# mathwrx/Decouple-and-Couple_Learning_in_Multi-Modal_Brain_Tumor_Segmentation

Hardware: AMD Instinct MI355X
Metric: training volumes/sec (4x128^3) (higher is better)
Workload: dtype bf16x3 forward (split-bf16 MFMA operands hi.hi+hi.lo+lo.hi: logits within 1e-3 of the fp32 reference) / bf16 data-gradient / bf16 weight-gradient MFMA operands; f32 accumulate, f32 storage, f32 master weights; 1 GPU; configs[1]: 1xMI355X, batch 2 per GPU, 4-modality 128^3 synthetic BraTS patches; fwd + softmax_dice + 4 sub-region/edge losses + bwd + Adam(amsgrad); random-init weights, dropout on; global_batch=2, parallelism=dp1, precision=bf16x3, dgrad_precision=bf16, wgrad_precision=bf16, mode=plan

## Files before the change

decouple-and-couple_learning_in_multi-modal_brain_tumor_segmentation_amd/csrc/attn.hip:

```cpp
#include "common.h"

#define AT_D 64
#define AT_TMAX 144
#define AT_QT 32
#define AT_LDK 68
#define AT_LDS 148

struct AttnArgs {
  const float* qkv; int64_t ld;
  float* o; int64_t ldo;
  const float* d_o;
  float* dqkv;
  int T, E, heads; float scale;
  const uint64_t* rng; uint64_t drop_off; float drop_p;
};

__device__ __forceinline__ f32x4 mfma4(float a, float b, f32x4 c) { return __builtin_amdgcn_mfma_f32_16x16x4f32(a, b, c, 0, 0, 0); }

__device__ __forceinline__ void at_load_tile(float* lds, const float* g, int64_t ld, int row0, int nrows, int valid_rows, int tid) {
  for (int i = tid; i < nrows * (AT_D / 4); i += 256) {
    const int r = i >> 4, c4 = (i & 15) * 4;
    float4 v = make_float4(0.f, 0.f, 0.f, 0.f);
    if (row0 + r < valid_rows) v = *reinterpret_cast<const float4*>(g + (int64_t)(row0 + r) * ld + c4);
    *reinterpret_cast<float4*>(lds + r * AT_LDK + c4) = v;
  }
}

__device__ __forceinline__ void at_scores(float* Ss, const float* As, const float* Bs, float alpha, int wave, int r, int kq) {
  for (int idx = wave; idx < 2 * 9; idx += 4) {
    const int mt = idx / 9, nt = idx % 9;
    f32x4 acc = {0.f, 0.f, 0.f, 0.f};
#pragma unroll
    for (int kk = 0; kk < AT_D / 4; ++kk)
      acc = mfma4(As[(mt * 16 + r) * AT_LDK + kk * 4 + kq], Bs[(nt * 16 + r) * AT_LDK + kk * 4 + kq], acc);
#pragma unroll
    for (int e = 0; e < 4; ++e) Ss[(mt * 16 + kq * 4 + e) * AT_LDS + nt * 16 + r] = acc[e] * alpha;
  }
}

__global__ __launch_bounds__(256) void attn_fwd_kernel(const AttnArgs a) {
  extern __shared__ float4 at_lds4[];
  float* Ks = reinterpret_cast<float*>(at_lds4);
  float* Vs = Ks + AT_TMAX * AT_LDK;
  float* Qs = Vs + AT_TMAX * AT_LDK;
// ... 30 lines not shown
        s[c] = p;
      }
    }
  }
  __syncthreads();
  for (int idx = wave; idx < 2 * 4; idx += 4) {
    const int mt = idx >> 2, nt = idx & 3;
    f32x4 acc = {0.f, 0.f, 0.f, 0.f};
#pragma unroll 4
    for (int kk = 0; kk < AT_TMAX / 4; ++kk)
      acc = mfma4(Ss[(mt * 16 + r) * AT_LDS + kk * 4 + kq], Vs[(kk * 4 + kq) * AT_LDK + nt * 16 + r], acc);
#pragma unroll
    for (int e = 0; e < 4; ++e) {
      const int q = q0 + mt * 16 + kq * 4 + e;
      if (q < T) a.o[((int64_t)z * T + q) * a.ldo + h * AT_D + nt * 16 + r] = acc[e];
    }
  }
}

__global__ __launch_bounds__(256) void attn_bwd_kernel(const AttnArgs a) {
  extern __shared__ float4 at_lds4[];
  float* Ks = reinterpret_cast<float*>(at_lds4);
  float* Vs = Ks + AT_TMAX * AT_LDK;
  float* Qs = Vs + AT_TMAX * AT_LDK;
  float* Gs = Qs + AT_QT * AT_LDK;
  float* Ss = Gs + AT_QT * AT_LDK;
  float* Ds = Ss + AT_QT * AT_LDS;
  const int tid = threadIdx.x, lane = tid & 63, wave = tid >> 6, r = lane & 15, kq = lane >> 4;
  const int zh = blockIdx.x, z = zh / a.heads, h = zh % a.heads, T = a.T;
  const float* base = a.qkv + (int64_t)z * T * a.ld + h * AT_D;
// ... 3 lines not shown
  at_load_tile(Vs, base + 2 * a.E, a.ld, 0, AT_TMAX, T, tid);
  f32x4 dk[9], dv[9];
#pragma unroll
  for (int i = 0; i < 9; ++i) { dk[i] = (f32x4){0.f, 0.f, 0.f, 0.f}; dv[i] = (f32x4){0.f, 0.f, 0.f, 0.f}; }
  const float inv_keep = a.drop_p > 0.f ? 1.f / (1.f - a.drop_p) : 1.f;
  for (int q0 = 0; q0 < T; q0 += AT_QT) {
    __syncthreads();
    at_load_tile(Qs, base, a.ld, q0, AT_QT, T, tid);
    at_load_tile(Gs, gbase, a.ldo, q0, AT_QT, T, tid);
    __syncthreads();
    at_scores(Ss, Qs, Ks, a.scale, wave, r, kq);
    at_scores(Ds, Gs, Vs, 1.f, wave, r, kq);
    __syncthreads();
    for (int rr = 0; rr < 8; ++rr) {
      const int row = wave * 8 + rr;
      float* s = Ss + row * AT_LDS; float* d = Ds + row * AT_LDS;
      const bool live = q0 + row < T;
      float v[3], g[3]; float mx = -INFINITY;
#pragma unroll
      for (int i = 0; i < 3; ++i) { const int c = lane + 64 * i; v[i] = c < T ? s[c] : -INFINITY; mx = fmaxf(mx, v[i]); }
      mx = wave_max(mx);
      float sum = 0.f;
#pragma unroll
      for (int i = 0; i < 3; ++i) { v[i] = (lane + 64 * i) < T ? expf(v[i] - mx) : 0.f; sum += v[i]; }
      const float inv = 1.f / wave_sum(sum);
      float dot = 0.f; float m[3];
#pragma unroll
      for (int i = 0; i < 3; ++i) {
        const int c = lane + 64 * i;
        v[i] *= inv; m[i] = 1.f;
        if (a.drop_p > 0.f && c < T)
          m[i] = cwf_rng_u01(a.rng, a.drop_off + ((uint64_t)zh * T + (q0 + row)) * T + c) >= a.drop_p ? inv_keep : 0.f;
        g[i] = c < T ? d[c] * m[i] : 0.f;
        dot += g[i] * v[i];
      }
      dot = wave_sum(dot);
#pragma unroll
      for (int i = 0; i < 3; ++i) {
        const int c = lane + 64 * i;
        if (c < AT_TMAX) {
          s[c] = live ? v[i] * m[i] : 0.f;
          d[c] = live ? v[i] * (g[i] - dot) * a.scale : 0.f;
        }
      }
    }
    __syncthreads();
#pragma unroll
    for (int mt = 0; mt < 9; ++mt) {
#pragma unroll
      for (int kk = 0; kk < AT_QT / 4; ++kk) {
        const int q = kk * 4 + kq;
        dv[mt] = mfma4(Ss[q * AT_LDS + mt * 16 + r], Gs[q * AT_LDK + wave * 16 + r], dv[mt]);
        dk[mt] = mfma4(Ds[q * AT_LDS + mt * 16 + r], Qs[q * AT_LDK + wave * 16 + r], dk[mt]);
      }
    }
    for (int idx = wave; idx < 2 * 4; idx += 4) {
      const int mt = idx >> 2, nt = idx & 3;
      f32x4 acc = {0.f, 0.f, 0.f, 0.f};
#pragma unroll 4
// ... 6 lines not shown
      }
    }
  }
#pragma unroll
  for (int mt = 0; mt < 9; ++mt)
#pragma unroll
    for (int e = 0; e < 4; ++e) {
      const int key = mt * 16 + kq * 4 + e;
      if (key < T) {
        dbase[(int64_t)key * a.ld + a.E + wave * 16 + r] = dk[mt][e];
        dbase[(int64_t)key * a.ld + 2 * a.E + wave * 16 + r] = dv[mt][e];
      }
    }
}

static int at_check(const float* qkv, int64_t ld, int Z, int T, int E, int heads) {
  if (!qkv || Z <= 0 || T <= 0 || heads <= 0 || E != heads * AT_D || ld < 3 * (int64_t)E || (ld & 3) || ((uintptr_t)qkv & 15)) return CWF_E_BADARG;
  if (T > AT_TMAX || (int64_t)Z * heads > 65535) return CWF_E_TOOLARGE;
  return 0;
}

static void at_set_lds(const void* fn, size_t bytes) {
  static bool done[2][64] = {};
  static const void* fns[2] = {nullptr, nullptr};
  int dev = 0; (void)hipGetDevice(&dev);
  int slot = (fns[0] == fn || fns[0] == nullptr) ? 0 : 1;
  fns[slot] = fn;
  if (dev < 0 || dev >= 64 || !done[slot][dev]) {
    (void)hipFuncSetAttribute(fn, hipFuncAttributeMaxDynamicSharedMemorySize, (int)bytes);
    if (dev >= 0 && dev < 64) done[slot][dev] = true;
  }
}

extern "C" int cwf_attn_fwd(const float* qkv, int64_t ld, float* o, int64_t ldo, int Z, int T, int E, int heads, float scale,
                            const uint64_t* rng, uint64_t drop_off, float drop_p, void* stream) {
  int rc = at_check(qkv, ld, Z, T, E, heads); if (rc) return rc;
  if (!o || ldo < E || (drop_p > 0.f && !rng) || drop_p < 0.f || drop_p >= 1.f) return CWF_E_BADARG;
  AttnArgs a{qkv, ld, o, ldo, nullptr, nullptr, T, E, heads, scale, rng, drop_off, drop_p};
  const size_t lds = sizeof(float) * (2 * AT_TMAX * AT_LDK + AT_QT * AT_LDK + AT_QT * AT_LDS);
  at_set_lds(reinterpret_cast<const void*>(&attn_fwd_kernel), lds);
  hipLaunchKernelGGL(attn_fwd_kernel, dim3(cdiv(T, AT_QT), Z * heads), dim3(256), lds, cwf_stream(stream), a);
  CWF_LAUNCH_CHECK();
  return 0;
}

extern "C" int cwf_attn_bwd(const float* qkv, int64_t ld, const float* d_o, int64_t ldo, float* dqkv, int Z, int T, int E, int heads,
                            float scale, const uint64_t* rng, uint64_t drop_off, float drop_p, void* stream) {
  int rc = at_check(qkv, ld, Z, T, E, heads); if (rc) return rc;
  if (!d_o || !dqkv || ldo < E || (ldo & 3) || ((uintptr_t)d_o & 15) || (drop_p > 0.f && !rng) || drop_p < 0.f || drop_p >= 1.f) return CWF_E_BADARG;
  AttnArgs a{qkv, ld, nullptr, ldo, d_o, dqkv, T, E, heads, scale, rng, drop_off, drop_p};
  const size_t lds = sizeof(float) * (2 * AT_TMAX * AT_LDK + 2 * AT_QT * AT_LDK + 2 * AT_QT * AT_LDS);
  at_set_lds(reinterpret_cast<const void*>(&attn_bwd_kernel), lds);
  hipLaunchKernelGGL(attn_bwd_kernel, dim3(Z * heads), dim3(256), lds, cwf_stream(stream), a);
  CWF_LAUNCH_CHECK();
  return 0;
}
```

decouple-and-couple_learning_in_multi-modal_brain_tumor_segmentation_amd/csrc/tokens.hip:

```cpp
#include "common.h"

__global__ void window_to_tokens_kernel(const float* __restrict__ x, int x_ldc, float* __restrict__ tok,
                                        int D, int H, int W, int C, int p0, int p1, int p2, int64_t total) {
  const int64_t idx = (int64_t)blockIdx.x * blockDim.x + threadIdx.x;
  if (idx >= total) return;
  const int E = C * p0 * p1 * p2;
  const int T = (D / p0) * (H / p1) * (W / p2);
  const int f = (int)(idx % E); const int64_t bt = idx / E;
  const int t = (int)(bt % T); const int b = (int)(bt / T);
  int ff = f; const int k = ff % p2; ff /= p2; const int j = ff % p1; ff /= p1; const int i = ff % p0; const int c = ff / p0;
  int tt = t; const int tw = tt % (W / p2); tt /= (W / p2); const int th = tt % (H / p1); const int td = tt / (H / p1);
  const int d = td * p0 + i, h = th * p1 + j, w = tw * p2 + k;
  tok[idx] = x[((((int64_t)b * D + d) * H + h) * W + w) * x_ldc + c];
}

__global__ void tokens_to_window_kernel(const float* __restrict__ tok, float* __restrict__ x, int x_ldc,
                                        int D, int H, int W, int C, int p0, int p1, int p2, int accumulate, int64_t total) {
  const int64_t idx = (int64_t)blockIdx.x * blockDim.x + threadIdx.x;
  if (idx >= total) return;
  const int c = (int)(idx % C); int64_t v = idx / C;
  const int w = (int)(v % W); v /= W; const int h = (int)(v % H); v /= H; const int d = (int)(v % D); const int b = (int)(v / D);
  const int E = C * p0 * p1 * p2;
  const int T = (D / p0) * (H / p1) * (W / p2);
  const int t = ((d / p0) * (H / p1) + h / p1) * (W / p2) + w / p2;
// ... 332 lines not shown
    float4 v = *reinterpret_cast<const float4*>(src + e);
    if (scat) *reinterpret_cast<float4*>(scat + o + e) = v;
    if (gated) {
      const float4 g = *reinterpret_cast<const float4*>(gate + b * gate_bs + e);
      v.x *= g.x; v.y *= g.y; v.z *= g.z; v.w *= g.w;
      *reinterpret_cast<float4*>(gated + o + e) = v;
    }
  }
}

struct ScatBwdArgs {
  const float* dgated; const float* dscat; const float* feats; const int32_t* inv; const int32_t* index;
  const float* rows; int64_t rows_ld, rows_bs; const float* gate; int64_t gate_bs; const float* dgate_extra; int64_t extra_bs;
  float* drows; int64_t drows_ld, drows_bs; float* dgate; int64_t dgate_bs; int T, k, E;
};
__global__ __launch_bounds__(1024) void scatter_bwd_kernel(const ScatBwdArgs a) {
  const int b = blockIdx.y, E = a.E, T = a.T;
  if ((int)blockIdx.x < a.k) {
    if (threadIdx.x >= 128) return;
    const int j = blockIdx.x;
    const int t = min(max(a.index[(int64_t)b * a.k + j], 0), T - 1);
    const int64_t o = ((int64_t)b * T + t) * E;
    for (int e = threadIdx.x * 4; e < E; e += 512) {
      float4 v = make_float4(0.f, 0.f, 0.f, 0.f);
      if (a.dgated) {
        const float4 d = *reinterpret_cast<const float4*>(a.dgated + o + e);
        const float4 g = *reinterpret_cast<const float4*>(a.gate + b * a.gate_bs + e);
        v = make_float4(d.x * g.x, d.y * g.y, d.z * g.z, d.w * g.w);
      }
      if (a.dscat) { const float4 s = *reinterpret_cast<const float4*>(a.dscat + o + e); v.x += s.x; v.y += s.y; v.z += s.z; v.w += s.w; }
      *reinterpret_cast<float4*>(a.drows + b * a.drows_bs + (int64_t)j * a.drows_ld + e) = v;
    }
    return;
  }
  __shared__ float red[16][64];
  const int w = threadIdx.x >> 6, lane = threadIdx.x & 63;
  const int c = (blockIdx.x - a.k) * 64 + lane;
  float acc = 0.f;
  if (c < E && a.dgated) {
    for (int t0 = w; t0 < T; t0 += 64) {
      float d[4], s[4];
#pragma unroll
      for (int u = 0; u < 4; ++u) {
        const int t = t0 + 16 * u;
        d[u] = 0.f; s[u] = 0.f;
        if (t < T) {
          const int j = a.inv[(int64_t)b * T + t];
          d[u] = a.dgated[((int64_t)b * T + t) * E + c];
          s[u] = j >= 0 ? a.rows[b * a.rows_bs + (int64_t)j * a.rows_ld + c] : a.feats[((int64_t)b * T + t) * E + c];
        }
      }
#pragma unroll
      for (int u = 0; u < 4; ++u) acc += d[u] * s[u];
    }
  }
  red[w][lane] = acc;
  __syncthreads();
  if (w == 0 && c < E) {
    float tsum = 0.f;
#pragma unroll
    for (int i = 0; i < 16; ++i) tsum += red[i][lane];
    if (a.dgate_extra) tsum += a.dgate_extra[b * a.extra_bs + c];
    a.dgate[b * a.dgate_bs + c] = tsum;
  }
}

struct TokGradArgs {
  const float* dgated; const float* dscat; const float* gate; int64_t gate_bs;
  const int32_t* inv_p; const int32_t* inv_q;
  const float* dseq_p; int64_t dseq_p_bs; const float* dseq_q; int64_t dseq_q_bs;
  uint64_t drop_off_p, drop_off_q; float p; const uint64_t* rng;
  float* dfeats; int B, T, k, E;
};
__global__ __launch_bounds__(128) void token_grad_kernel(const TokGradArgs a) {
  const int t = blockIdx.x, b = blockIdx.y, E = a.E, T = a.T, k = a.k;
  const int jp = a.inv_p[(int64_t)b * T + t];
  const int jq = a.inv_q ? a.inv_q[(int64_t)b * T + t] : -1;
  const int64_t o = ((int64_t)b * T + t) * E;
// ... 92 lines not shown
  a.k = k; a.E = E; a.pe_odd = pe_odd; a.p = p; a.rng = rng;
  hipLaunchKernelGGL(gather_multi_kernel, dim3(k + 1, B, njobs), dim3(128), 0, cwf_stream(stream), a);
  CWF_LAUNCH_CHECK();
  return 0;
}

extern "C" int cwf_scatter_inv(const float* feats, const int32_t* inv, const float* rows, int64_t rows_ld, int64_t rows_bs,
                               const float* gate, int64_t gate_bs, float* gated, float* scat, int B, int T, int E, void* stream) {
  if (!feats || !inv || !rows || (!gated && !scat) || (gated && !gate) || B <= 0 || T <= 0 || (E & 3) || (rows_ld & 3) || (rows_bs & 3) || (gate_bs & 3))
    return CWF_E_BADARG;
  hipLaunchKernelGGL(scatter_inv_kernel, dim3(T, B), dim3(128), 0, cwf_stream(stream), feats, inv, rows, rows_ld, rows_bs, gate, gate_bs, gated, scat, T, E);
  CWF_LAUNCH_CHECK();
  return 0;
}

extern "C" int cwf_scatter_bwd(const float* dgated, const float* dscat, const float* feats, const int32_t* inv, const int32_t* index,
                               const float* rows, int64_t rows_ld, int64_t rows_bs, const float* gate, int64_t gate_bs,
                               const float* dgate_extra, int64_t extra_bs, float* drows, int64_t drows_ld, int64_t drows_bs,
                               float* dgate, int64_t dgate_bs, int B, int T, int k, int E, void* stream) {
  if (!feats || !inv || !index || !rows || !drows || !dgate || B <= 0 || T <= 0 || k <= 0 || (E & 63)) return CWF_E_BADARG;
  if (dgated && !gate) return CWF_E_BADARG;
  if ((rows_ld | rows_bs | gate_bs | drows_ld | drows_bs) & 3) return CWF_E_BADARG;
  ScatBwdArgs a{dgated, dscat, feats, inv, index, rows, rows_ld, rows_bs, gate, gate_bs, dgate_extra, extra_bs, drows, drows_ld, drows_bs,
                dgate, dgate_bs, T, k, E};
  hipLaunchKernelGGL(scatter_bwd_kernel, dim3(k + E / 64, B), dim3(1024), 0, cwf_stream(stream), a);
  CWF_LAUNCH_CHECK();
  return 0;
}

extern "C" int cwf_token_grad(const float* dgated, const float* dscat, const float* gate, int64_t gate_bs,
                              const int32_t* inv_p, const int32_t* inv_q, const float* dseq_p, int64_t dseq_p_bs,
                              const float* dseq_q, int64_t dseq_q_bs, const uint64_t* rng, uint64_t drop_off_p, uint64_t drop_off_q, float p,
                              float* dfeats, int B, int T, int k, int E, void* stream) {
  if (!inv_p || !dseq_p || !dfeats || B <= 0 || T <= 0 || k <= 0 || (E & 3) || (inv_q && !dseq_q) || (dgated && !gate)) return CWF_E_BADARG;
  if ((p > 0.f && !rng) || p < 0.f || p >= 1.f || ((gate_bs | dseq_p_bs | dseq_q_bs) & 3)) return CWF_E_BADARG;
  TokGradArgs a{dgated, dscat, gate, gate_bs, inv_p, inv_q, dseq_p, dseq_p_bs, dseq_q, dseq_q_bs, drop_off_p, drop_off_q, p, rng, dfeats, B, T, k, E};
  hipLaunchKernelGGL(token_grad_kernel, dim3(T, B), dim3(128), 0, cwf_stream(stream), a);
  CWF_LAUNCH_CHECK();
  return 0;
}
// ... 127 lines not shown
```

decouple-and-couple_learning_in_multi-modal_brain_tumor_segmentation_amd/cwf/_lib.py:

```python
from __future__ import annotations

import ctypes as C
import os

_HERE = os.path.dirname(os.path.abspath(__file__))
LIB_PATH = os.path.join(_HERE, "libcwf_hip.so")

P = C.c_void_p
I = C.c_int
L = C.c_int64
F = C.c_float
U = C.c_uint32
U64 = C.c_uint64
D = C.c_double

SIGNATURES = {
    "cwf_version": [],
    "cwf_conv": [P, P],
    "cwf_conv_x16_ok": [I, I, I, I, I, I, I],
    "cwf_debug_wsd": [I],
    "cwf_debug_wsd_launches": [],
    "cwf_wgrad": [P, P, P],
    "cwf_debug_wgrad_bf16_plan": [P, P],
    "cwf_debug_wgrad_bf16_name": [I],
# ... 42 lines not shown
                       F, P, P, F, P],
    "cwf_wgrad_reduce_batched": [P, I, P],
    "cwf_dropout_mask": [P, L, F, F, C.c_uint64, C.c_uint64, P],
    "cwf_mul": [P, P, P, L, P],
    "cwf_add": [P, P, P, L, P],
    "cwf_channel_scale": [P, I, P, P, I, I, L, I, P],
    "cwf_copy_strided": [P, I, P, I, L, I, P],
    "cwf_add3": [P, P, P, P, L, P],
    "cwf_bcast3": [P, P, L, P],
    "cwf_stats_channel_sum": [P, P, I, I, P],
    "cwf_gemm_ex": [P, P],
    "cwf_debug_gemm_panel": [I],
    "cwf_debug_gemm_panel_launches": [],
    "cwf_attn_fwd": [P, L, P, L, I, I, I, I, F, P, U64, F, P],
    "cwf_attn_bwd": [P, L, P, L, P, I, I, I, I, F, P, U64, F, P],
    "cwf_ln_pair_fwd": [P, P, I, P, P, P, P, P, P, P, I, I, F, P],
    "cwf_ln_pair_bwd": [P, P, P, P, P, I, P, P, P, P, P, P, P, P, P, I, I, I, P],
    "cwf_gelu_bwd_drop": [P, P, P, L, P, U64, F, P],
    "cwf_token_scores2": [P, P, L, P, L, P, P, I, I, I, P],
    "cwf_topk_inv": [P, P, P, P, P, P, I, I, I, P],
    "cwf_index_inv": [P, P, I, I, I, P],
    "cwf_gather_multi": [P, I, I, I, I, F, P, F, P],
    "cwf_scatter_inv": [P, P, P, L, L, P, L, P, P, I, I, I, P],
    "cwf_scatter_bwd": [P, P, P, P, P, P, L, L, P, L, P, L, P, L, L, P, L, I, I, I, I, P],
    "cwf_token_grad": [P, P, P, L, P, P, P, L, P, L, P, U64, U64, F, P, I, I, I, I, P],
    "cwf_head_grad": [P, P, P, P, L, P, P, I, I, P],
    "cwf_dice_ce_finalize_multi": [P, P, P, P, I, I, L, I, P],
    "cwf_head_loss_sums": [P, I, I, P, P, P, I, I, I, I, I, P],
    "cwf_head_loss_bwd": [P, I, I, P, P, P, P, P, I, P, I, I, I, I, I, P],
    "cwf_head_loss_bwd_ex": [P, I, I, P, P, P, P, P, I, I, P, I, I, I, I, I, P],
    "cwf_ln_pair_fwd_g": [P, P, I, P, I, P, P, P, I, I, F, P],
    "cwf_ln_pair_bwd_g": [P, P, P, P, P, I, P, I, P, P, P, I, I, I, P],
    "cwf_token_scores2_g": [P, P, P, I, I, P, P, I, I, I, P],
    "cwf_head_grad_g": [P, P, P, P, L, P, P, I, I, I, P],
    "cwf_window_to_tokens_g": [P, I, P, I, I, I, I, I, I, I, I, I, P],
    "cwf_tokens_to_window_g": [P, P, I, I, I, I, I, I, I, I, I, I, P],
    "cwf_cat3_channels": [P, P, P, P, L, I, P],
    "cwf_stitch_windows": [P, P, I, P],
    "cwf_argmax_dice": [P, L, L, L, P, P, P, I, L, P],
# ... 173 lines not shown

WINDOW_MAX_STARTS = 128


class WindowGrid(C.Structure):
    _fields_ = [("B", I), ("S", I * 3), ("r", I * 3), ("n", I * 3), ("start", (I * WINDOW_MAX_STARTS) * 3)]


class WindowBox(C.Structure):
    _fields_ = [("full", I * 3), ("lo", I * 3)]


NORM_WS_DOUBLES = 2568
GRADNORM_WS_DOUBLES = 1024
RULE_ADAMW, RULE_SGD = 1, 2
RESTYPE_INT64 = {"cwf_debug_wsd_launches", "cwf_debug_gemm_panel_launches", "cwf_wgrad_partial_floats", "cwf_wgrad_slab_floats", "cwf_hausdorff_workspace", "cwf_components_workspace",
                 "cwf_lesionwise_workspace", "cwf_surface_metrics_workspace", "cwf_lesionwise_ex_workspace", "cwf_signed_distance_workspace",
                 "cwf_topk_ce_workspace", "cwf_focal_workspace", "cwf_lovasz_workspace", "cwf_class_locations_workspace", "cwf_nonzero_box_workspace"}
LOCATIONS_TILE = 16384
NONZERO_BOX_TILE = 4096

_lib = None


class CwfError(RuntimeError):
    pass


def load():
    global _lib
    if _lib is not None:
# ... 22 lines not shown
```

decouple-and-couple_learning_in_multi-modal_brain_tumor_segmentation_amd/cwf/kernels.py:

```python
from __future__ import annotations

import contextlib
import ctypes
import math
import threading

import numpy as np
import torch

from . import _lib
from . import packing as pk

_f32 = torch.float32
REGION_MASKS = (0b1110, 0b1010, 0b1000)
FOCAL_DEFAULTS = dict(fn=0.7, fp=0.3, exponent=0.75, smooth=1e-5, gamma=2.0, ce_ratio=1.0, class_weight=(1.0, 1.0, 1.0, 1.0))


def check_focal_params(posmasks, fn=0.7, fp=0.3, exponent=0.75, smooth=1e-5, gamma=2.0, ce_ratio=1.0, class_weight=None):
    masks = tuple(int(m) for m in posmasks)
    if len(masks) > 8:
        raise ValueError("focal loss: at most 8 regions, got %d" % len(masks))
    if any(m <= 0 or m > 15 for m in masks):
        raise ValueError("focal loss: a region is a non-zero bitmask over classes 0..3, got %r" % (posmasks,))
    fn, fp, exponent, smooth, gamma, ce_ratio = (float(v) for v in (fn, fp, exponent, smooth, gamma, ce_ratio))
# ... 822 lines not shown
        return dx, dx2

    def attn_fwd(self, qkv, z, t, heads, drop=None):
        e = qkv.shape[1] // 3
        o = torch.empty((z * t, e), dtype=_f32, device=qkv.device)
        off, p = (drop[0], drop[1]) if drop else (0, 0.0)
        self._call("cwf_attn_fwd", qkv.data_ptr(), qkv.stride(0), o.data_ptr(), e, z, t, e, heads, float((e // heads) ** -0.5),
                   self.rng(qkv.device).data_ptr(), off, float(p), self._stream())
        return o

    def attn_bwd(self, qkv, d_o, z, t, heads, drop=None):
        e = qkv.shape[1] // 3
        assert d_o.is_contiguous()
        dqkv = torch.empty_like(qkv)
        off, p = (drop[0], drop[1]) if drop else (0, 0.0)
        self._call("cwf_attn_bwd", qkv.data_ptr(), qkv.stride(0), d_o.data_ptr(), e, dqkv.data_ptr(), z, t, e, heads,
                   float((e // heads) ** -0.5), self.rng(qkv.device).data_ptr(), off, float(p), self._stream())
        return dqkv

    def gelu_bwd_drop(self, z, dh, drop=None):
        dz = torch.empty_like(z)
        off, p = (drop[0], drop[1]) if drop else (0, 0.0)
        self._call("cwf_gelu_bwd_drop", z.data_ptr(), dh.data_ptr(), dz.data_ptr(), z.numel(), self.rng(z.device).data_ptr(), off, float(p), self._stream())
        return dz

    def token_scores2(self, feats, q1, q2=None):
        b, t, e = feats.shape
        s1 = torch.empty((b, t), dtype=_f32, device=feats.device)
        s2 = torch.empty((b, t), dtype=_f32, device=feats.device) if q2 is not None else None
        if isinstance(q1, (list, tuple)):
            G = len(q1)
            t1 = (ctypes.c_void_p * G)(*[q.data_ptr() for q in q1])
# ... 960 lines not shown
```

include/cwf_hip.h:

```cpp
#ifndef CWF_HIP_H
#define CWF_HIP_H
#include <stdint.h>
#ifdef __cplusplus
extern "C" {
#endif

#define CWF_E_BADARG   (-1)
#define CWF_E_TOOLARGE (-2)
#define CWF_E_ALIGN    (-3)

int cwf_version(void);
const char* cwf_arch(void);

enum { CWF_CONV3_S1 = 0, CWF_CONV3_S2 = 1, CWF_CONV1 = 2, CWF_CONVT2 = 3, CWF_CONV3_S2_DGRAD = 4, CWF_CONVT2_DGRAD = 5 };
enum { CWF_FP32 = 0, CWF_BF16X3 = 1, CWF_BF16 = 2 };

struct cwf_conv_args {
  int op, precision;
  const float* x; int x_ldc; const void* wpk; const float* bias; float* y; int y_ldc;
  const float* in_scale; const float* in_shift; float in_slope;
  const float* residual; int r_ldc; const float* out_scale; double* stats;
  const float* nb_x; int nb_ldc; const float* nb_scale; const float* nb_shift; float nb_slope;
  const void* x16; const void* zero16; void* y16;
  const float* w_raw;
// ... 77 lines not shown
  float* C2;
  float* rowsum; int rowsum_acc;
  const uint64_t* rng;
  uint64_t a_drop_off, a_drop_n; float a_drop_p, a_drop_p2;
  uint64_t c_drop_off, c_drop_n; float c_drop_p, c_drop_p2;
  const float* B_tab[4]; const float* bias_tab[4]; float* C_tab[4]; float* rowsum_tab[4];
};
int cwf_gemm_ex(const struct cwf_gemm_args* args , void* stream);
int cwf_debug_gemm_panel(int v);
long long cwf_debug_gemm_panel_launches(void);

int cwf_attn_fwd(const float* qkv, int64_t ld, float* o, int64_t ldo, int Z, int T, int E, int heads, float scale,
                 const uint64_t* rng, uint64_t drop_off, float drop_p, void* stream);
int cwf_attn_bwd(const float* qkv, int64_t ld, const float* d_o, int64_t ldo, float* dqkv, int Z, int T, int E, int heads,
                 float scale, const uint64_t* rng, uint64_t drop_off, float drop_p, void* stream);

int cwf_ln_pair_fwd(const float* x, const float* x2, int perm_T, const float* g1, const float* b1, const float* g2, const float* b2,
                    float* ya, float* yb, float* stats, int rows, int E, float eps, void* stream);
struct cwf_ln_group_params { const float* g1[4]; const float* b1[4]; const float* g2[4]; const float* b2[4];
                             float* dg1[4]; float* db1[4]; float* dg2[4]; float* db2[4]; };
int cwf_ln_pair_fwd_g(const float* x, const float* x2, int perm_T, const struct cwf_ln_group_params* h_params, int groups,
                      float* ya, float* yb, float* stats, int rows, int E, float eps, void* stream);
int cwf_ln_pair_bwd_g(const float* dy, const float* da, const float* db, const float* x, const float* x2, int perm_T,
                      const struct cwf_ln_group_params* h_params, int groups, const float* stats, float* dx, float* dx2,
                      int rows, int E, int accumulate_params, void* stream);
int cwf_ln_pair_bwd(const float* dy, const float* da, const float* db, const float* x, const float* x2, int perm_T,
                    const float* g1, const float* g2, const float* stats, float* dx, float* dx2,
                    float* dg1, float* db1, float* dg2, float* db2, int rows, int E, int accumulate_params, void* stream);
int cwf_gelu_bwd_drop(const float* z, const float* dh, float* dz, int64_t n, const uint64_t* rng, uint64_t off, float p, void* stream);

// ... 29 lines not shown
                        float* s1, float* s2, int B, int T, int E, void* stream);
int cwf_topk_inv(const float* score0, int32_t* index0, int32_t* inv0, const float* score1, int32_t* index1, int32_t* inv1,
                 int B, int T, int k, void* stream);
int cwf_index_inv(const int32_t* index, int32_t* inv, int B, int T, int k, void* stream);
struct cwf_gather_job { const float* feats; const int32_t* index; const float* head; float* out;
                        int64_t head_bstride, out_bstride; int T; uint64_t drop_off;
                        const float* head_g[4]; int group_B;  };
int cwf_gather_multi(const struct cwf_gather_job* jobs , int njobs, int B, int k, int E, float pe_odd,
                     const uint64_t* rng, float p, void* stream);
int cwf_scatter_inv(const float* feats, const int32_t* inv, const float* rows, int64_t rows_ld, int64_t rows_bs,
                    const float* gate, int64_t gate_bs, float* gated, float* scat, int B, int T, int E, void* stream);
int cwf_scatter_bwd(const float* dgated, const float* dscat, const float* feats, const int32_t* inv, const int32_t* index,
                    const float* rows, int64_t rows_ld, int64_t rows_bs, const float* gate, int64_t gate_bs,
                    const float* dgate_extra, int64_t extra_bs, float* drows, int64_t drows_ld, int64_t drows_bs,
                    float* dgate, int64_t dgate_bs, int B, int T, int k, int E, void* stream);
int cwf_token_grad(const float* dgated, const float* dscat, const float* gate, int64_t gate_bs,
                   const int32_t* inv_p, const int32_t* inv_q, const float* dseq_p, int64_t dseq_p_bs,
                   const float* dseq_q, int64_t dseq_q_bs, const uint64_t* rng, uint64_t drop_off_p, uint64_t drop_off_q, float p,
                   float* dfeats, int B, int T, int k, int E, void* stream);
int cwf_head_grad(const float* a1, const float* c1, const float* a2, const float* c2, int64_t bstride,
                  float* out1, float* out2, int B, int E, void* stream);
int cwf_head_grad_g(const float* a1, const float* c1, const float* a2, const float* c2, int64_t bstride,
                    float* const* h_out1, float* const* h_out2, int groups, int group_B, int E, void* stream);
int cwf_window_to_tokens_g(const float* x, int x_ldc, float* tok, int groups, int B, int D, int H, int W, int C,
                           int p0, int p1, int p2, void* stream);
int cwf_tokens_to_window_g(const float* tok, float* x, int x_ldc, int groups, int B, int D, int H, int W, int C,
                           int p0, int p1, int p2, void* stream);
int cwf_cat3_channels(const float* x0, const float* x1, const float* x2, float* y, int64_t nvox, int C, void* stream);

int cwf_upsample_softmax(const float* logit, int l_ldc, float* prob, int N, int D, int H, int W, int C, int scale,
// ... 236 lines not shown
```

Measured before the change: 122.3 volumes/s.

## Split attention backward across query tiles and widen scatter-gate grad kernel

Attention backward previously ran one block per (batch, head) and looped serially over query tiles. It is now split into two kernels. A rows kernel gets one block per query tile, with configurable wave count, and computes the softmax/dropout gradient rows and dQ, writing P and dS to a global workspace. A keys kernel then reduces dK/dV per 16-key tile. Separately, the scatter backward dgate reduction gets a narrower-column kernel with more blocks and vector loads. The aim is more parallelism on a small-grid stage, at the cost of extra workspace traffic and one more launch.

```diff
diff --git a/decouple-and-couple_learning_in_multi-modal_brain_tumor_segmentation_amd/csrc/attn.hip b/decouple-and-couple_learning_in_multi-modal_brain_tumor_segmentation_amd/csrc/attn.hip
--- a/decouple-and-couple_learning_in_multi-modal_brain_tumor_segmentation_amd/csrc/attn.hip
+++ b/decouple-and-couple_learning_in_multi-modal_brain_tumor_segmentation_amd/csrc/attn.hip
@@ -17,8 +17,9 @@
 
 __device__ __forceinline__ f32x4 mfma4(float a, float b, f32x4 c) { return __builtin_amdgcn_mfma_f32_16x16x4f32(a, b, c, 0, 0, 0); }
 
+template <int NT = 256>
 __device__ __forceinline__ void at_load_tile(float* lds, const float* g, int64_t ld, int row0, int nrows, int valid_rows, int tid) {
-  for (int i = tid; i < nrows * (AT_D / 4); i += 256) {
+  for (int i = tid; i < nrows * (AT_D / 4); i += NT) {
     const int r = i >> 4, c4 = (i & 15) * 4;
     float4 v = make_float4(0.f, 0.f, 0.f, 0.f);
     if (row0 + r < valid_rows) v = *reinterpret_cast<const float4*>(g + (int64_t)(row0 + r) * ld + c4);
@@ -26,8 +27,9 @@
   }
 }
 
+template <int NW = 4>
 __device__ __forceinline__ void at_scores(float* Ss, const float* As, const float* Bs, float alpha, int wave, int r, int kq) {
-  for (int idx = wave; idx < 2 * 9; idx += 4) {
+  for (int idx = wave; idx < 2 * 9; idx += NW) {
     const int mt = idx / 9, nt = idx % 9;
     f32x4 acc = {0.f, 0.f, 0.f, 0.f};
 #pragma unroll
@@ -88,6 +90,38 @@
     for (int e = 0; e < 4; ++e) {
       const int q = q0 + mt * 16 + kq * 4 + e;
       if (q < T) a.o[((int64_t)z * T + q) * a.ldo + h * AT_D + nt * 16 + r] = acc[e];
+    }
+  }
+}
+
+__device__ __forceinline__ void at_bwd_row(const AttnArgs& a, float* s, float* d, int zh, int T, int qrow, int lane, float inv_keep) {
+#pragma clang fp contract(off)
+  const bool live = qrow < T;
+  float v[3], g[3]; float mx = -INFINITY;
+#pragma unroll
+  for (int i = 0; i < 3; ++i) { const int c = lane + 64 * i; v[i] = c < T ? s[c] : -INFINITY; mx = fmaxf(mx, v[i]); }
+  mx = wave_max(mx);
+  float sum = 0.f;
+#pragma unroll
+  for (int i = 0; i < 3; ++i) { v[i] = (lane + 64 * i) < T ? expf(v[i] - mx) : 0.f; sum += v[i]; }
+  const float inv = 1.f / wave_sum(sum);
+  float dot = 0.f; float m[3];
+#pragma unroll
+  for (int i = 0; i < 3; ++i) {
+    const int c = lane + 64 * i;
+    v[i] *= inv; m[i] = 1.f;
+    if (a.drop_p > 0.f && c < T)
+      m[i] = cwf_rng_u01(a.rng, a.drop_off + ((uint64_t)zh * T + qrow) * T + c) >= a.drop_p ? inv_keep : 0.f;
+    g[i] = c < T ? d[c] * m[i] : 0.f;
+    dot = fmaf(g[i], v[i], dot);
+  }
+  dot = wave_sum(dot);
+#pragma unroll
+  for (int i = 0; i < 3; ++i) {
+    const int c = lane + 64 * i;
+    if (c < AT_TMAX) {
+      s[c] = live ? v[i] * m[i] : 0.f;
+      d[c] = live ? v[i] * (g[i] - dot) * a.scale : 0.f;
     }
   }
 }
@@ -121,35 +155,7 @@
     __syncthreads();
     for (int rr = 0; rr < 8; ++rr) {
       const int row = wave * 8 + rr;
-      float* s = Ss + row * AT_LDS; float* d = Ds + row * AT_LDS;
-      const bool live = q0 + row < T;
-      float v[3], g[3]; float mx = -INFINITY;
-#pragma unroll
-      for (int i = 0; i < 3; ++i) { const int c = lane + 64 * i; v[i] = c < T ? s[c] : -INFINITY; mx = fmaxf(mx, v[i]); }
-      mx = wave_max(mx);
-      float sum = 0.f;
-#pragma unroll
-      for (int i = 0; i < 3; ++i) { v[i] = (lane + 64 * i) < T ? expf(v[i] - mx) : 0.f; sum += v[i]; }
-      const float inv = 1.f / wave_sum(sum);
-      float dot = 0.f; float m[3];
-#pragma unroll
-      for (int i = 0; i < 3; ++i) {
-        const int c = lane + 64 * i;
-        v[i] *= inv; m[i] = 1.f;
-        if (a.drop_p > 0.f && c < T)
-          m[i] = cwf_rng_u01(a.rng, a.drop_off + ((uint64_t)zh * T + (q0 + row)) * T + c) >= a.drop_p ? inv_keep : 0.f;
-        g[i] = c < T ? d[c] * m[i] : 0.f;
-        dot += g[i] * v[i];
-      }
-      dot = wave_sum(dot);
-#pragma unroll
-      for (int i = 0; i < 3; ++i) {
-        const int c = lane + 64 * i;
-        if (c < AT_TMAX) {
-          s[c] = live ? v[i] * m[i] : 0.f;
-          d[c] = live ? v[i] * (g[i] - dot) * a.scale : 0.f;
-        }
-      }
+      at_bwd_row(a, Ss + row * AT_LDS, Ds + row * AT_LDS, zh, T, q0 + row, lane, inv_keep);
     }
     __syncthreads();
 #pragma unroll
@@ -186,6 +192,94 @@
     }
 }
 
+struct AttnSplitArgs { AttnArgs a; float* pd; float* ds; int tpad; };
+
+template <int NW>
+__global__ __launch_bounds__(NW * 64) void attn_bwd_rows_kernel(const AttnSplitArgs sa) {
+  const AttnArgs& a = sa.a;
+  extern __shared__ float4 at_lds4[];
+  float* Ks = reinterpret_cast<float*>(at_lds4);
+  float* Vs = Ks + AT_TMAX * AT_LDK;
+  float* Qs = Vs + AT_TMAX * AT_LDK;
+  float* Gs = Qs + AT_QT * AT_LDK;
+  float* Ss = Gs + AT_QT * AT_LDK;
+  float* Ds = Ss + AT_QT * AT_LDS;
+  constexpr int NT = NW * 64;
+  const int tid = threadIdx.x, lane = tid & 63, wave = tid >> 6, r = lane & 15, kq = lane >> 4;
+  const int zh = blockIdx.y, z = zh / a.heads, h = zh % a.heads, T = a.T, q0 = blockIdx.x * AT_QT;
+  const float* base = a.qkv + (int64_t)z * T * a.ld + h * AT_D;
+  const float* gbase = a.d_o + (int64_t)z * T * a.ldo + h * AT_D;
+  float* dbase = a.dqkv + (int64_t)z * T * a.ld + h * AT_D;
+  at_load_tile<NT>(Ks, base + a.E, a.ld, 0, AT_TMAX, T, tid);
+  at_load_tile<NT>(Vs, base + 2 * a.E, a.ld, 0, AT_TMAX, T, tid);
+  at_load_tile<NT>(Qs, base, a.ld, q0, AT_QT, T, tid);
+  at_load_tile<NT>(Gs, gbase, a.ldo, q0, AT_QT, T, tid);
+  const float inv_keep = a.drop_p > 0.f ? 1.f / (1.f - a.drop_p) : 1.f;
+  __syncthreads();
+  at_scores<NW>(Ss, Qs, Ks, a.scale, wave, r, kq);
+  at_scores<NW>(Ds, Gs, Vs, 1.f, wave, r, kq);
+  __syncthreads();
+  for (int row = wave; row < AT_QT; row += NW)
+    at_bwd_row(a, Ss + row * AT_LDS, Ds + row * AT_LDS, zh, T, q0 + row, lane, inv_keep);
+  __syncthreads();
+  {
+    float* pd = sa.pd + ((int64_t)zh * sa.tpad + q0) * AT_TMAX;
+    float* ds = sa.ds + ((int64_t)zh * sa.tpad + q0) * AT_TMAX;
+    for (int i = tid; i < AT_QT * (AT_TMAX / 4); i += NT) {
+      const int row = i / (AT_TMAX / 4), c4 = (i % (AT_TMAX / 4)) * 4;
+      *reinterpret_cast<float4*>(pd + row * AT_TMAX + c4) = *reinterpret_cast<const float4*>(Ss + row * AT_LDS + c4);
+      *reinterpret_cast<float4*>(ds + row * AT_TMAX + c4) = *reinterpret_cast<const float4*>(Ds + row * AT_LDS + c4);
+    }
+  }
+  for (int idx = wave; idx < 2 * 4; idx += NW) {
+    const int mt = idx >> 2, nt = idx & 3;
+    f32x4 acc = {0.f, 0.f, 0.f, 0.f};
+#pragma unroll 4
+    for (int kk = 0; kk < AT_TMAX / 4; ++kk)
+      acc = mfma4(Ds[(mt * 16 + r) * AT_LDS + kk * 4 + kq], Ks[(kk * 4 + kq) * AT_LDK + nt * 16 + r], acc);
+#pragma unroll
+    for (int e = 0; e < 4; ++e) {
+      const int q = q0 + mt * 16 + kq * 4 + e;
+      if (q < T) dbase[(int64_t)q * a.ld + nt * 16 + r] = acc[e];
+    }
+  }
+}
+
+__global__ __launch_bounds__(256) void attn_bwd_keys_kernel(const AttnSplitArgs sa) {
+  const AttnArgs& a = sa.a;
+  const int tid = threadIdx.x, lane = tid & 63, wave = tid >> 6, r = lane & 15, kq = lane >> 4;
+  const int zh = blockIdx.y, z = zh / a.heads, h = zh % a.heads, T = a.T, kt = blockIdx.x;
+  if (kt * 16 >= T) return;
+  const float* qb = a.qkv + (int64_t)z * T * a.ld + h * AT_D + wave * 16 + r;
+  const float* gb = a.d_o + (int64_t)z * T * a.ldo + h * AT_D + wave * 16 + r;
+  const float* pd = sa.pd + (int64_t)zh * sa.tpad * AT_TMAX + kt * 16 + r;
+  const float* ds = sa.ds + (int64_t)zh * sa.tpad * AT_TMAX + kt * 16 + r;
+  float* dbase = a.dqkv + (int64_t)z * T * a.ld + h * AT_D;
+  f32x4 dk = {0.f, 0.f, 0.f, 0.f}, dv = {0.f, 0.f, 0.f, 0.f};
+  for (int q0 = 0; q0 < T; q0 += AT_QT) {
+    float p[AT_QT / 4], s[AT_QT / 4], g[AT_QT / 4], x[AT_QT / 4];
+#pragma unroll
+    for (int kk = 0; kk < AT_QT / 4; ++kk) {
+      const int q = q0 + kk * 4 + kq;
+      p[kk] = pd[(int64_t)q * AT_TMAX]; s[kk] = ds[(int64_t)q * AT_TMAX];
+      g[kk] = q < T ? gb[(int64_t)q * a.ldo] : 0.f; x[kk] = q < T ? qb[(int64_t)q * a.ld] : 0.f;
+    }
+#pragma unroll
+    for (int kk = 0; kk < AT_QT / 4; ++kk) {
+      dv = mfma4(p[kk], g[kk], dv);
+      dk = mfma4(s[kk], x[kk], dk);
+    }
+  }
+#pragma unroll
+  for (int e = 0; e < 4; ++e) {
+    const int key = kt * 16 + kq * 4 + e;
+    if (key < T) {
+      dbase[(int64_t)key * a.ld + a.E + wave * 16 + r] = dk[e];
+      dbase[(int64_t)key * a.ld + 2 * a.E + wave * 16 + r] = dv[e];
+    }
+  }
+}
+
 static int at_check(const float* qkv, int64_t ld, int Z, int T, int E, int heads) {
   if (!qkv || Z <= 0 || T <= 0 || heads <= 0 || E != heads * AT_D || ld < 3 * (int64_t)E || (ld & 3) || ((uintptr_t)qkv & 15)) return CWF_E_BADARG;
   if (T > AT_TMAX || (int64_t)Z * heads > 65535) return CWF_E_TOOLARGE;
@@ -193,14 +287,16 @@
 }
 
 static void at_set_lds(const void* fn, size_t bytes) {
-  static bool done[2][64] = {};
-  static const void* fns[2] = {nullptr, nullptr};
+  constexpr int SLOTS = 8;
+  static bool done[SLOTS][64] = {};
+  static const void* fns[SLOTS] = {};
   int dev = 0; (void)hipGetDevice(&dev);
-  int slot = (fns[0] == fn || fns[0] == nullptr) ? 0 : 1;
-  fns[slot] = fn;
-  if (dev < 0 || dev >= 64 || !done[slot][dev]) {
+  int slot = 0;
+  while (slot < SLOTS && fns[slot] != fn && fns[slot] != nullptr) ++slot;
+  if (slot < SLOTS) fns[slot] = fn;
+  if (slot >= SLOTS || dev < 0 || dev >= 64 || !done[slot][dev]) {
     (void)hipFuncSetAttribute(fn, hipFuncAttributeMaxDynamicSharedMemorySize, (int)bytes);
-    if (dev >= 0 && dev < 64) done[slot][dev] = true;
+    if (slot < SLOTS && dev >= 0 && dev < 64) done[slot][dev] = true;
   }
 }
 
@@ -227,3 +323,47 @@
   CWF_LAUNCH_CHECK();
   return 0;
 }
+
+static int g_attn_split = 1;
+static int g_attn_split_waves = 8;
+static long long g_attn_split_launches = 0;
+extern "C" int cwf_debug_attn_split(int v) { const int old = g_attn_split; g_attn_split = v; return old; }
+extern "C" int cwf_debug_attn_split_waves(int v) {
+  const int old = g_attn_split_waves;
+  if (v == 4 || v == 8 || v == 16) g_attn_split_waves = v;
+  return old;
+}
+extern "C" long long cwf_debug_attn_split_launches() { return g_attn_split_launches; }
+
+template <int NW>
+static void at_launch_rows(const AttnSplitArgs& sa, int Z, size_t lds, void* stream) {
+  at_set_lds(reinterpret_cast<const void*>(&attn_bwd_rows_kernel<NW>), lds);
+  hipLaunchKernelGGL(attn_bwd_rows_kernel<NW>, dim3(cdiv(sa.a.T, AT_QT), Z * sa.a.heads), dim3(NW * 64), lds, cwf_stream(stream), sa);
+}
+
+extern "C" int64_t cwf_attn_bwd_ws_bytes(int Z, int T, int heads) {
+  if (Z <= 0 || T <= 0 || heads <= 0) return 0;
+  return (int64_t)2 * Z * heads * (cdiv(T, AT_QT) * AT_QT) * AT_TMAX * sizeof(float);
+}
+
+extern "C" int cwf_attn_bwd_ws(const float* qkv, int64_t ld, const float* d_o, int64_t ldo, float* dqkv, int Z, int T, int E, int heads,
+                               float scale, const uint64_t* rng, uint64_t drop_off, float drop_p, void* ws, int64_t ws_bytes, void* stream) {
+  int rc = at_check(qkv, ld, Z, T, E, heads); if (rc) return rc;
+  if (!d_o || !dqkv || ldo < E || (ldo & 3) || ((uintptr_t)d_o & 15) || (drop_p > 0.f && !rng) || drop_p < 0.f || drop_p >= 1.f) return CWF_E_BADARG;
+  if (!ws || ((uintptr_t)ws & 15) || ws_bytes < cwf_attn_bwd_ws_bytes(Z, T, heads)) return CWF_E_BADARG;
+  if (g_attn_split == 0) return cwf_attn_bwd(qkv, ld, d_o, ldo, dqkv, Z, T, E, heads, scale, rng, drop_off, drop_p, stream);
+  AttnSplitArgs sa;
+  sa.a = AttnArgs{qkv, ld, nullptr, ldo, d_o, dqkv, T, E, heads, scale, rng, drop_off, drop_p};
+  sa.tpad = cdiv(T, AT_QT) * AT_QT;
+  sa.pd = static_cast<float*>(ws);
+  sa.ds = sa.pd + (int64_t)Z * heads * sa.tpad * AT_TMAX;
+  const size_t lds = sizeof(float) * (2 * AT_TMAX * AT_LDK + 2 * AT_QT * AT_LDK + 2 * AT_QT * AT_LDS);
+  if (g_attn_split_waves == 4) at_launch_rows<4>(sa, Z, lds, stream);
+  else if (g_attn_split_waves == 16) at_launch_rows<16>(sa, Z, lds, stream);
+  else at_launch_rows<8>(sa, Z, lds, stream);
+  CWF_LAUNCH_CHECK();
+  hipLaunchKernelGGL(attn_bwd_keys_kernel, dim3(AT_TMAX / 16, Z * heads), dim3(256), 0, cwf_stream(stream), sa);
+  CWF_LAUNCH_CHECK();
+  ++g_attn_split_launches;
+  return 0;
+}
diff --git a/decouple-and-couple_learning_in_multi-modal_brain_tumor_segmentation_amd/csrc/tokens.hip b/decouple-and-couple_learning_in_multi-modal_brain_tumor_segmentation_amd/csrc/tokens.hip
--- a/decouple-and-couple_learning_in_multi-modal_brain_tumor_segmentation_amd/csrc/tokens.hip
+++ b/decouple-and-couple_learning_in_multi-modal_brain_tumor_segmentation_amd/csrc/tokens.hip
@@ -370,23 +370,27 @@
   const float* rows; int64_t rows_ld, rows_bs; const float* gate; int64_t gate_bs; const float* dgate_extra; int64_t extra_bs;
   float* drows; int64_t drows_ld, drows_bs; float* dgate; int64_t dgate_bs; int T, k, E;
 };
+__device__ __forceinline__ void scat_bwd_drows(const ScatBwdArgs& a, int b, int j, int tid, int nt) {
+#pragma clang fp contract(off)
+  const int E = a.E, T = a.T;
+  const int t = min(max(a.index[(int64_t)b * a.k + j], 0), T - 1);
+  const int64_t o = ((int64_t)b * T + t) * E;
+  for (int e = tid * 4; e < E; e += nt * 4) {
+    float4 v = make_float4(0.f, 0.f, 0.f, 0.f);
+    if (a.dgated) {
+      const float4 d = *reinterpret_cast<const float4*>(a.dgated + o + e);
+      const float4 g = *reinterpret_cast<const float4*>(a.gate + b * a.gate_bs + e);
+      v = make_float4(d.x * g.x, d.y * g.y, d.z * g.z, d.w * g.w);
+    }
+    if (a.dscat) { const float4 s = *reinterpret_cast<const float4*>(a.dscat + o + e); v.x += s.x; v.y += s.y; v.z += s.z; v.w += s.w; }
+    *reinterpret_cast<float4*>(a.drows + b * a.drows_bs + (int64_t)j * a.drows_ld + e) = v;
+  }
+}
+
 __global__ __launch_bounds__(1024) void scatter_bwd_kernel(const ScatBwdArgs a) {
   const int b = blockIdx.y, E = a.E, T = a.T;
   if ((int)blockIdx.x < a.k) {
-    if (threadIdx.x >= 128) return;
-    const int j = blockIdx.x;
-    const int t = min(max(a.index[(int64_t)b * a.k + j], 0), T - 1);
-    const int64_t o = ((int64_t)b * T + t) * E;
-    for (int e = threadIdx.x * 4; e < E; e += 512) {
-      float4 v = make_float4(0.f, 0.f, 0.f, 0.f);
-      if (a.dgated) {
-        const float4 d = *reinterpret_cast<const float4*>(a.dgated + o + e);
-        const float4 g = *reinterpret_cast<const float4*>(a.gate + b * a.gate_bs + e);
-        v = make_float4(d.x * g.x, d.y * g.y, d.z * g.z, d.w * g.w);
-      }
-      if (a.dscat) { const float4 s = *reinterpret_cast<const float4*>(a.dscat + o + e); v.x += s.x; v.y += s.y; v.z += s.z; v.w += s.w; }
-      *reinterpret_cast<float4*>(a.drows + b * a.drows_bs + (int64_t)j * a.drows_ld + e) = v;
-    }
+    if (threadIdx.x < 128) scat_bwd_drows(a, b, blockIdx.x, threadIdx.x, 128);
     return;
   }
   __shared__ float red[16][64];
@@ -407,7 +411,10 @@
         }
       }
 #pragma unroll
-      for (int u = 0; u < 4; ++u) acc += d[u] * s[u];
+      for (int u = 0; u < 4; ++u) {
+#pragma clang fp contract(off)
+        acc = acc + d[u] * s[u];
+      }
     }
   }
   red[w][lane] = acc;
@@ -418,6 +425,52 @@
     for (int i = 0; i < 16; ++i) tsum += red[i][lane];
     if (a.dgate_extra) tsum += a.dgate_extra[b * a.extra_bs + c];
     a.dgate[b * a.dgate_bs + c] = tsum;
+  }
+}
+
+template <int COLS, int VEC>
+__global__ __launch_bounds__(16 * COLS / VEC) void scatter_bwd_wide_kernel(const ScatBwdArgs a) {
+  constexpr int NT = 16 * COLS / VEC, CT = COLS / VEC, R = 16;
+  typedef float fv __attribute__((ext_vector_type(VEC)));
+  const int b = blockIdx.y, E = a.E, T = a.T;
+  if ((int)blockIdx.x < a.k) { scat_bwd_drows(a, b, blockIdx.x, threadIdx.x, NT); return; }
+  __shared__ float red[16][COLS];
+  const int w = threadIdx.x / CT, ct = threadIdx.x % CT;
+  const int c0 = (blockIdx.x - a.k) * COLS;
+  const int c = c0 + ct * VEC;
+  fv acc = 0.f;
+  if (a.dgated) {
+    const int64_t row0 = (int64_t)b * T;
+    for (int t0 = w; t0 < T; t0 += 16 * R) {
+      int j[R]; fv d[R], s[R];
+#pragma unroll
+      for (int u = 0; u < R; ++u) { const int t = t0 + 16 * u; j[u] = t < T ? a.inv[row0 + t] : -1; }
+#pragma unroll
+      for (int u = 0; u < R; ++u) {
+        const int t = t0 + 16 * u;
+        d[u] = 0.f; s[u] = 0.f;
+        if (t < T) {
+          d[u] = *reinterpret_cast<const fv*>(a.dgated + (row0 + t) * E + c);
+          s[u] = *reinterpret_cast<const fv*>(j[u] >= 0 ? a.rows + b * a.rows_bs + (int64_t)j[u] * a.rows_ld + c : a.feats + (row0 + t) * E + c);
+        }
+      }
+#pragma unroll
+      for (int u = 0; u < R; ++u) {
+#pragma clang fp contract(off)
+        acc = acc + d[u] * s[u];
+      }
+    }
+  }
+#pragma unroll
+  for (int i = 0; i < VEC; ++i) red[w][ct * VEC + i] = acc[i];
+  __syncthreads();
+  if ((int)threadIdx.x < COLS) {
+    const int col = threadIdx.x;
+    float tsum = 0.f;
+#pragma unroll
+    for (int i = 0; i < 16; ++i) tsum += red[i][col];
+    if (a.dgate_extra) tsum += a.dgate_extra[b * a.extra_bs + c0 + col];
+    a.dgate[b * a.dgate_bs + c0 + col] = tsum;
   }
 }
 
@@ -540,6 +593,14 @@
   return 0;
 }
 
+constexpr int SCB_WIDE_COLS = 16;
+static int g_scatter_bwd = 1;
+extern "C" int cwf_debug_scatter_bwd(int v) {
+  const int old = g_scatter_bwd;
+  if (v == 0 || v == 1 || v == 8 || v == 16 || v == 32) g_scatter_bwd = v;
+  return old;
+}
+
 extern "C" int cwf_scatter_bwd(const float* dgated, const float* dscat, const float* feats, const int32_t* inv, const int32_t* index,
                                const float* rows, int64_t rows_ld, int64_t rows_bs, const float* gate, int64_t gate_bs,
                                const float* dgate_extra, int64_t extra_bs, float* drows, int64_t drows_ld, int64_t drows_bs,
@@ -549,7 +610,12 @@
   if ((rows_ld | rows_bs | gate_bs | drows_ld | drows_bs) & 3) return CWF_E_BADARG;
   ScatBwdArgs a{dgated, dscat, feats, inv, index, rows, rows_ld, rows_bs, gate, gate_bs, dgate_extra, extra_bs, drows, drows_ld, drows_bs,
                 dgate, dgate_bs, T, k, E};
-  hipLaunchKernelGGL(scatter_bwd_kernel, dim3(k + E / 64, B), dim3(1024), 0, cwf_stream(stream), a);
+  const bool aligned = !(((uintptr_t)dgated | (uintptr_t)feats | (uintptr_t)rows) & 15);
+  const int cols = !aligned ? 0 : g_scatter_bwd == 1 ? SCB_WIDE_COLS : g_scatter_bwd;
+  if (cols == 8) hipLaunchKernelGGL((scatter_bwd_wide_kernel<8, 2>), dim3(k + E / 8, B), dim3(64), 0, cwf_stream(stream), a);
+  else if (cols == 16) hipLaunchKernelGGL((scatter_bwd_wide_kernel<16, 4>), dim3(k + E / 16, B), dim3(64), 0, cwf_stream(stream), a);
+  else if (cols == 32) hipLaunchKernelGGL((scatter_bwd_wide_kernel<32, 4>), dim3(k + E / 32, B), dim3(128), 0, cwf_stream(stream), a);
+  else hipLaunchKernelGGL(scatter_bwd_kernel, dim3(k + E / 64, B), dim3(1024), 0, cwf_stream(stream), a);
   CWF_LAUNCH_CHECK();
   return 0;
 }
diff --git a/decouple-and-couple_learning_in_multi-modal_brain_tumor_segmentation_amd/cwf/_lib.py b/decouple-and-couple_learning_in_multi-modal_brain_tumor_segmentation_amd/cwf/_lib.py
--- a/decouple-and-couple_learning_in_multi-modal_brain_tumor_segmentation_amd/cwf/_lib.py
+++ b/decouple-and-couple_learning_in_multi-modal_brain_tumor_segmentation_amd/cwf/_lib.py
@@ -80,6 +80,11 @@
     "cwf_debug_gemm_panel_launches": [],
     "cwf_attn_fwd": [P, L, P, L, I, I, I, I, F, P, U64, F, P],
     "cwf_attn_bwd": [P, L, P, L, P, I, I, I, I, F, P, U64, F, P],
+    "cwf_attn_bwd_ws": [P, L, P, L, P, I, I, I, I, F, P, U64, F, P, L, P],
+    "cwf_attn_bwd_ws_bytes": [I, I, I],
+    "cwf_debug_attn_split": [I],
+    "cwf_debug_attn_split_waves": [I],
+    "cwf_debug_attn_split_launches": [],
     "cwf_ln_pair_fwd": [P, P, I, P, P, P, P, P, P, P, I, I, F, P],
     "cwf_ln_pair_bwd": [P, P, P, P, P, I, P, P, P, P, P, P, P, P, P, I, I, I, P],
     "cwf_gelu_bwd_drop": [P, P, P, L, P, U64, F, P],
@@ -89,6 +94,7 @@
     "cwf_gather_multi": [P, I, I, I, I, F, P, F, P],
     "cwf_scatter_inv": [P, P, P, L, L, P, L, P, P, I, I, I, P],
     "cwf_scatter_bwd": [P, P, P, P, P, P, L, L, P, L, P, L, P, L, L, P, L, I, I, I, I, P],
+    "cwf_debug_scatter_bwd": [I],
     "cwf_token_grad": [P, P, P, L, P, P, P, L, P, L, P, U64, U64, F, P, I, I, I, I, P],
     "cwf_head_grad": [P, P, P, P, L, P, P, I, I, P],
     "cwf_dice_ce_finalize_multi": [P, P, P, P, I, I, L, I, P],
@@ -292,7 +298,7 @@
 NORM_WS_DOUBLES = 2568
 GRADNORM_WS_DOUBLES = 1024
 RULE_ADAMW, RULE_SGD = 1, 2
-RESTYPE_INT64 = {"cwf_debug_wsd_launches", "cwf_debug_gemm_panel_launches", "cwf_wgrad_partial_floats", "cwf_wgrad_slab_floats", "cwf_hausdorff_workspace", "cwf_components_workspace",
+RESTYPE_INT64 = {"cwf_debug_wsd_launches", "cwf_debug_gemm_panel_launches", "cwf_debug_attn_split_launches", "cwf_attn_bwd_ws_bytes", "cwf_wgrad_partial_floats", "cwf_wgrad_slab_floats", "cwf_hausdorff_workspace", "cwf_components_workspace",
                  "cwf_lesionwise_workspace", "cwf_surface_metrics_workspace", "cwf_lesionwise_ex_workspace", "cwf_signed_distance_workspace",
                  "cwf_topk_ce_workspace", "cwf_focal_workspace", "cwf_lovasz_workspace", "cwf_class_locations_workspace", "cwf_nonzero_box_workspace"}
 LOCATIONS_TILE = 16384
diff --git a/decouple-and-couple_learning_in_multi-modal_brain_tumor_segmentation_amd/cwf/kernels.py b/decouple-and-couple_learning_in_multi-modal_brain_tumor_segmentation_amd/cwf/kernels.py
--- a/decouple-and-couple_learning_in_multi-modal_brain_tumor_segmentation_amd/cwf/kernels.py
+++ b/decouple-and-couple_learning_in_multi-modal_brain_tumor_segmentation_amd/cwf/kernels.py
@@ -860,8 +860,10 @@
         assert d_o.is_contiguous()
         dqkv = torch.empty_like(qkv)
         off, p = (drop[0], drop[1]) if drop else (0, 0.0)
-        self._call("cwf_attn_bwd", qkv.data_ptr(), qkv.stride(0), d_o.data_ptr(), e, dqkv.data_ptr(), z, t, e, heads,
-                   float((e // heads) ** -0.5), self.rng(qkv.device).data_ptr(), off, float(p), self._stream())
+        nbytes = int(self.lib.cwf_attn_bwd_ws_bytes(z, t, heads))
+        ws = self.workspace("attn_bwd", nbytes // 4, qkv.device)
+        self._call("cwf_attn_bwd_ws", qkv.data_ptr(), qkv.stride(0), d_o.data_ptr(), e, dqkv.data_ptr(), z, t, e, heads,
+                   float((e // heads) ** -0.5), self.rng(qkv.device).data_ptr(), off, float(p), ws.data_ptr(), ws.numel() * 4, self._stream())
         return dqkv
 
     def gelu_bwd_drop(self, z, dh, drop=None):
diff --git a/include/cwf_hip.h b/include/cwf_hip.h
--- a/include/cwf_hip.h
+++ b/include/cwf_hip.h
@@ -115,6 +115,12 @@
                  const uint64_t* rng, uint64_t drop_off, float drop_p, void* stream);
 int cwf_attn_bwd(const float* qkv, int64_t ld, const float* d_o, int64_t ldo, float* dqkv, int Z, int T, int E, int heads,
                  float scale, const uint64_t* rng, uint64_t drop_off, float drop_p, void* stream);
+int64_t cwf_attn_bwd_ws_bytes(int Z, int T, int heads);
+int cwf_attn_bwd_ws(const float* qkv, int64_t ld, const float* d_o, int64_t ldo, float* dqkv, int Z, int T, int E, int heads,
+                    float scale, const uint64_t* rng, uint64_t drop_off, float drop_p, void* ws, int64_t ws_bytes, void* stream);
+int cwf_debug_attn_split(int v);
+int cwf_debug_attn_split_waves(int v);
+long long cwf_debug_attn_split_launches(void);
 
 int cwf_ln_pair_fwd(const float* x, const float* x2, int perm_T, const float* g1, const float* b1, const float* g2, const float* b2,
                     float* ya, float* yb, float* stats, int rows, int E, float eps, void* stream);
@@ -174,6 +180,7 @@
                     const float* rows, int64_t rows_ld, int64_t rows_bs, const float* gate, int64_t gate_bs,
                     const float* dgate_extra, int64_t extra_bs, float* drows, int64_t drows_ld, int64_t drows_bs,
                     float* dgate, int64_t dgate_bs, int B, int T, int k, int E, void* stream);
+int cwf_debug_scatter_bwd(int v);
 int cwf_token_grad(const float* dgated, const float* dscat, const float* gate, int64_t gate_bs,
                    const int32_t* inv_p, const int32_t* inv_q, const float* dseq_p, int64_t dseq_p_bs,
                    const float* dseq_q, int64_t dseq_q_bs, const uint64_t* rng, uint64_t drop_off_p, uint64_t drop_off_q, float p,
```

Measured after the change: 123.9 volumes/s (median of 6 runs). 1.01x the previous value.
